# mstksg/hamilton

Measured on AMD Instinct MI355X. Metric: RK4 phase-space steps/sec (ensemble), higher is better.
Workload: dtype f64

## Files before the change

hamilton_amd/csrc/hamk_codegen.cpp:

```cpp
#include "hamk_internal.h"

#include <algorithm>
#include <array>
#include <cmath>
#include <cstdio>
#include <cstring>
#include <functional>
#include <map>
#include <set>
#include <sstream>

namespace hamk_host {

static std::string lit(double c) {
  if (std::isnan(c)) return "hamk::quiet_nan()";
  if (std::isinf(c)) return c > 0 ? "__builtin_inf()" : "(-__builtin_inf())";
  char buf[64];
  std::snprintf(buf, sizeof buf, "%a", c);
  std::string s(buf);
  if (c < 0 || std::signbit(c)) s = "(" + s + ")";
  return s;
}

static const char* unary_name(int op) {
// ... 414 lines not shown
        acc(p.a, 'a', aI + " * fa" + I + " + " + bI + " * (faa" + I + " * " + tanr(p.a) + " + fab" + I + " * " + tanr(p.b) + ")");
        acc(p.a, 'b', bI + " * fa" + I);
        acc(p.b, 'a', aI + " * fb" + I + " + " + bI + " * (fab" + I + " * " + tanr(p.a) + " + fbb" + I + " * " + tanr(p.b) + ")");
        acc(p.b, 'b', bI + " * fb" + I);
        break;
      case HAMK_OP_SIN: {
        const std::string sl = std::to_string(r.slot[i]);
        acc(p.a, 'a', aI + " * tcr.c[" + sl + "] - " + bI + " * tcr.s[" + sl + "] * " + tanr(p.a));
        acc(p.a, 'b', bI + " * tcr.c[" + sl + "]");
      } break;
      case HAMK_OP_COS: {
        const std::string sl = std::to_string(r.slot[i]);
        acc(p.a, 'a', "-(" + aI + " * tcr.s[" + sl + "] + " + bI + " * tcr.c[" + sl + "] * " + tanr(p.a) + ")");
        acc(p.a, 'b', "-(" + bI + " * tcr.s[" + sl + "])");
      } break;
      default:
        acc(p.a, 'a', aI + " * g" + I + " + " + bI + " * h" + I + " * " + tanr(p.a));
        acc(p.a, 'b', bI + " * g" + I);
        break;
    }
  }
  for (int j = 0; j < d.n; ++j) o << "    dT[" << j << "] = -aq" << j << "; (void)bq" << j << ";\n";
  o << "  }\n";
}

int distinct_jacobian_entries(const SystemDesc& d) {
  const int n = d.n, nops = (int)d.f_ops.size();
  enum : long long { ZERO = 0, ONE = 1 };
  std::map<std::array<long long, 4>, long long> table;
  long long next = 2;
  auto node = [&](long long kind, long long a, long long b, long long c) -> long long {
    const std::array<long long, 4> key = {kind, a, b, c};
    auto it = table.find(key);
    if (it != table.end()) return it->second;
    table[key] = next;
    return next++;
  };
  auto add = [&](long long a, long long b) { if (a == ZERO) return b; if (b == ZERO) return a; return node(1, std::min(a, b), std::max(a, b), 0); };
  auto neg = [&](long long a) { return a == ZERO ? (long long)ZERO : node(2, a, 0, 0); };
  auto scale = [&](long long factor_kind, long long factor_id, long long a) {
    if (a == ZERO) return (long long)ZERO;
    return node(3, factor_kind * (1LL << 40) + factor_id, a, 0);
  };
  std::vector<std::vector<long long>> g(nops, std::vector<long long>(n, ZERO));
  for (int i = 0; i < nops; ++i) {
    const hamk_op& p = d.f_ops[i];
    switch (p.op) {
      case HAMK_OP_CONST: break;
      case HAMK_OP_INPUT: g[i][p.a] = ONE; break;
      case HAMK_OP_ADD: for (int j = 0; j < n; ++j) g[i][j] = add(g[p.a][j], g[p.b][j]); break;
      case HAMK_OP_SUB: for (int j = 0; j < n; ++j) g[i][j] = add(g[p.a][j], neg(g[p.b][j])); break;
      case HAMK_OP_NEG: for (int j = 0; j < n; ++j) g[i][j] = neg(g[p.a][j]); break;
      case HAMK_OP_MUL: {
        const bool ca = d.f_ops[p.a].op == HAMK_OP_CONST, cb = d.f_ops[p.b].op == HAMK_OP_CONST;
        for (int j = 0; j < n; ++j) {
          const long long t1 = cb ? (long long)ZERO : scale(ca ? 5 : 4, ca ? (long long)std::hash<double>{}(d.f_ops[p.a].c) & ((1LL << 40) - 1) : p.a, g[p.b][j]);
          const long long t2 = ca ? (long long)ZERO : scale(cb ? 5 : 4, cb ? (long long)std::hash<double>{}(d.f_ops[p.b].c) & ((1LL << 40) - 1) : p.b, g[p.a][j]);
          g[i][j] = add(t1, t2);
        }
      } break;
      case HAMK_OP_DIV: case HAMK_OP_POW: case HAMK_OP_ATAN2:
        for (int j = 0; j < n; ++j) g[i][j] = (g[p.a][j] == ZERO && g[p.b][j] == ZERO) ? (long long)ZERO : node(6, i, g[p.a][j], g[p.b][j]);
        break;
      default:
        for (int j = 0; j < n; ++j) g[i][j] = scale(7 + p.op, p.a, g[p.a][j]);
        break;
    }
  }
  std::set<long long> distinct;
  for (int k = 0; k < d.m; ++k)
    for (int j = 0; j < n; ++j)
      if (g[d.f_outs[k]][j] != ZERO) distinct.insert(g[d.f_outs[k]][j]);
  return (int)distinct.size();
}

long long forward_gradient_work(const SystemDesc& d) {
  const int n = d.n, nops = (int)d.f_ops.size();
  std::vector<std::vector<char>> sup(nops, std::vector<char>(n, 0));
  auto count = [&](const std::vector<char>& v) { long long c = 0; for (char x : v) c += x; return c; };
  long long work = 0;
  for (int i = 0; i < nops; ++i) {
    const hamk_op& p = d.f_ops[i];
    if (p.op == HAMK_OP_CONST) continue;
    if (p.op == HAMK_OP_INPUT) { sup[i][p.a] = 1; continue; }
    if (is_binary(p.op)) {
      long long both = 0, any = 0;
      for (int j = 0; j < n; ++j) { const char a = sup[p.a][j], b = sup[p.b][j]; sup[i][j] = a | b; both += a & b; any += a | b; }
      const bool ca = d.f_ops[p.a].op == HAMK_OP_CONST, cb = d.f_ops[p.b].op == HAMK_OP_CONST;
      if (p.op == HAMK_OP_ADD || p.op == HAMK_OP_SUB) work += both;
      else if (ca || cb) work += any;
      else work += count(sup[p.a]) + count(sup[p.b]);
    } else {
      sup[i] = sup[p.a];
      work += (p.op == HAMK_OP_NEG) ? 0 : count(sup[i]) + 2;
    }
  }
  return work;
}

namespace {
typedef std::vector<std::pair<int, int>> Mono;
typedef std::map<Mono, double> Poly;
struct SymFail {};

Mono mono_mul(const Mono& a, const Mono& b) {
  Mono r; size_t i = 0, j = 0;
  while (i < a.size() || j < b.size()) {
    if (j >= b.size() || (i < a.size() && a[i].first < b[j].first)) r.push_back(a[i++]);
    else if (i >= a.size() || b[j].first < a[i].first) r.push_back(b[j++]);
    else { r.push_back({a[i].first, a[i].second + b[j].second}); ++i; ++j; }
  }
  return r;
}
void poly_add(Poly& a, const Poly& b, double f = 1.0) {
  for (const auto& t : b) { a[t.first] += f * t.second; }
  if (a.size() > 20000) throw SymFail{};
}
Poly poly_mul(const Poly& a, const Poly& b) {
  Poly r;
  if (a.size() * b.size() > 200000) throw SymFail{};
  for (const auto& x : a) for (const auto& y : b) r[mono_mul(x.first, y.first)] += x.second * y.second;
  return r;
}
Poly poly_const(double c) { Poly p; if (c != 0.0) p[Mono{}] = c; return p; }
Poly poly_var(int v) { Poly p; p[Mono{{v, 1}}] = 1.0; return p; }
Poly poly_reduce(const Poly& a, int n, int hi = 1 << 30) {
  Poly cur = a;
  for (bool again = true; again;) {
    again = false;
    Poly next;
    for (const auto& t : cur) {
      int at = -1;
      for (size_t i = 0; i < t.first.size(); ++i)
        if (t.first[i].first >= n && t.first[i].first < hi && ((t.first[i].first - n) & 1) == 0 && t.first[i].second >= 2) { at = (int)i; break; }
      if (at < 0) { next[t.first] += t.second; continue; }
      again = true;
      Mono rest = t.first;
      const int sv = rest[at].first;
      rest[at].second -= 2;
      if (rest[at].second == 0) rest.erase(rest.begin() + at);
      next[rest] += t.second;
      next[mono_mul(rest, Mono{{sv + 1, 2}})] -= t.second;
    }
    cur.swap(next);
    if (cur.size() > 20000) throw SymFail{};
  }
  return cur;
}
void poly_prune(Poly& p, double scale) {
  for (auto it = p.begin(); it != p.end();) it = (std::fabs(it->second) <= 8.0 * 2.220446049250313e-16 * scale) ? p.erase(it) : std::next(it);
}
double poly_abs_sum(const Poly& p) { double s = 0.0; for (const auto& t : p) s += std::fabs(t.second); return s; }

struct SymK {
  bool ok = false;
  int n = 0;
  std::vector<Poly> k;
  std::vector<Poly> dT;
  int vbase = 0;
  bool dt_ok = false;
  long long sym_ops = 0, num_ops = 0, dt_ops = 0;
};

SymK symbolic_mass_matrix(const SystemDesc& d, const std::vector<int>& slot_operand) {
  SymK out;
  const int n = d.n, m = d.m, nops = (int)d.f_ops.size();
  out.n = n;
  if (n > 7 || d.mapping != HAMK_MAP_LANE) return out;
  std::vector<int> slot_of(nops, -1);
  for (size_t k = 0; k < slot_operand.size(); ++k) if (slot_operand[k] >= 0) slot_of[(size_t)slot_operand[k]] = (int)k;
  try {
    std::vector<Poly> V(nops);
    std::vector<std::vector<Poly>> G(nops, std::vector<Poly>(n));
    for (int i = 0; i < nops; ++i) {
      const hamk_op& p = d.f_ops[i];
      switch (p.op) {
        case HAMK_OP_CONST: V[i] = poly_const(p.c); break;
        case HAMK_OP_INPUT: V[i] = poly_var(p.a); G[i][p.a] = poly_const(1.0); break;
        case HAMK_OP_ADD: V[i] = V[p.a]; poly_add(V[i], V[p.b]); for (int j = 0; j < n; ++j) { G[i][j] = G[p.a][j]; poly_add(G[i][j], G[p.b][j]); } break;
        case HAMK_OP_SUB: V[i] = V[p.a]; poly_add(V[i], V[p.b], -1.0); for (int j = 0; j < n; ++j) { G[i][j] = G[p.a][j]; poly_add(G[i][j], G[p.b][j], -1.0); } break;
        case HAMK_OP_NEG: poly_add(V[i], V[p.a], -1.0); for (int j = 0; j < n; ++j) poly_add(G[i][j], G[p.a][j], -1.0); break;
        case HAMK_OP_MUL:
          V[i] = poly_reduce(poly_mul(V[p.a], V[p.b]), n);
          for (int j = 0; j < n; ++j) {
            if (!G[p.b][j].empty()) poly_add(G[i][j], poly_mul(V[p.a], G[p.b][j]));
            if (!G[p.a][j].empty()) poly_add(G[i][j], poly_mul(G[p.a][j], V[p.b]));
            G[i][j] = poly_reduce(G[i][j], n);
          }
          break;
        case HAMK_OP_DIV: {
          if (d.f_ops[p.b].op != HAMK_OP_CONST || d.f_ops[p.b].c == 0.0) throw SymFail{};
          const double r = 1.0 / d.f_ops[p.b].c;
          poly_add(V[i], V[p.a], r); for (int j = 0; j < n; ++j) poly_add(G[i][j], G[p.a][j], r);
        } break;
        case HAMK_OP_POWI: {
          if (p.b < 0 || p.b > 6) throw SymFail{};
          Poly acc = poly_const(1.0), dacc;
          for (int e = 0; e < p.b; ++e) { dacc = acc; acc = poly_reduce(poly_mul(acc, V[p.a]), n); }
          V[i] = acc;
          if (p.b >= 1) for (int j = 0; j < n; ++j) if (!G[p.a][j].empty()) { Poly t = poly_mul(dacc, G[p.a][j]); poly_add(G[i][j], t, (double)p.b); G[i][j] = poly_reduce(G[i][j], n); }
        } break;
        case HAMK_OP_SIN: case HAMK_OP_COS: {
          const int k = slot_of[p.a];
          if (k < 0) throw SymFail{};
          const int sv = n + 2 * k, cv = sv + 1;
          const bool is_sin = p.op == HAMK_OP_SIN;
          V[i] = poly_var(is_sin ? sv : cv);
          for (int j = 0; j < n; ++j)
            if (!G[p.a][j].empty()) { Poly t = poly_mul(poly_var(is_sin ? cv : sv), G[p.a][j]); poly_add(G[i][j], t, is_sin ? 1.0 : -1.0); G[i][j] = poly_reduce(G[i][j], n); }
        } break;
        default: throw SymFail{};
      }
    }
    out.k.resize((size_t)n * (n + 1) / 2);
    size_t e = 0;
    for (int a = 0; a < n; ++a)
      for (int b = a; b < n; ++b, ++e) {
        Poly acc;
        double scale = 0.0;
        int both = 0;
        for (int k = 0; k < m; ++k) {
          const Poly& ga = G[d.f_outs[k]][a];
          const Poly& gb = G[d.f_outs[k]][b];
          if (ga.empty() || gb.empty()) continue;
          ++both;
          Poly t = poly_mul(ga, gb);
          scale += std::fabs(d.inertia[k]) * poly_abs_sum(t);
          poly_add(acc, t, d.inertia[k]);
        }
        acc = poly_reduce(acc, n);
        poly_prune(acc, scale);
        out.num_ops += 2LL * both;
        for (const auto& t : acc) {
          int deg = 0; for (const auto& vp : t.first) deg += vp.second;
          out.sym_ops += deg + ((std::fabs(t.second) != 1.0 && deg > 0) ? 1 : 0);
        }
        if (acc.size() > 1) out.sym_ops += (long long)acc.size() - 1;
        if (acc.size() > 24) throw SymFail{};
        out.k[e] = acc;
      }
    out.ok = out.sym_ops < out.num_ops;
    if (out.ok) {
      const int nslots = (int)slot_operand.size();
      out.vbase = n + 2 * nslots;
      auto dvar = [&](int var, int i) -> Poly {
        if (var < n) return (var == i) ? poly_const(1.0) : Poly();
        const int k = (var - n) / 2;
        const Poly& arg = G[slot_operand[(size_t)k]][i];
        if (arg.empty()) return Poly();
        Poly r = poly_mul(poly_var(((var - n) & 1) ? var - 1 : var + 1), arg);
        if ((var - n) & 1) { Poly neg; poly_add(neg, r, -1.0); return neg; }
        return r;
      };
      out.dT.assign((size_t)n, Poly());
      bool fits = true;
      for (int i = 0; i < n && fits; ++i) {
        Poly acc;
        double scale = 0.0;
        size_t e2 = 0;
        for (int a = 0; a < n; ++a)
          for (int b = a; b < n; ++b, ++e2) {
            const double w = (a == b) ? -0.5 : -1.0;
            for (const auto& t : out.k[e2]) {
              for (size_t f = 0; f < t.first.size(); ++f) {
                const Poly dv = dvar(t.first[f].first, i);
                if (dv.empty()) continue;
                Mono rest = t.first;
                const double pw = (double)rest[f].second;
                rest[f].second -= 1;
                if (rest[f].second == 0) rest.erase(rest.begin() + (long)f);
                Mono vv = (a == b) ? Mono{{out.vbase + a, 2}} : Mono{{out.vbase + a, 1}, {out.vbase + b, 1}};
                Poly term; term[mono_mul(rest, vv)] = w * pw * t.second;
                Poly prod = poly_mul(term, dv);
                scale += poly_abs_sum(prod);
                poly_add(acc, prod);
              }
            }
          }
        acc = poly_reduce(acc, n, out.vbase);
        poly_prune(acc, scale);
        for (const auto& t : acc) { int deg = 0; for (const auto& vp : t.first) deg += vp.second; out.dt_ops += deg + 1; }
        if (acc.size() > 64) fits = false;
        out.dT[(size_t)i] = acc;
      }
      out.dt_ok = fits && out.dt_ops <= 12LL * n;
    }
  } catch (const SymFail&) { out.ok = false; out.dt_ok = false; }
  return out;
}

static std::string sym_poly_expr(const Poly& p, int n, int vbase) {
  std::ostringstream x;
  bool first = true;
  for (const auto& t : p) {
    std::ostringstream f;
    bool unit = true;
    for (const auto& vp : t.first)
      for (int r = 0; r < vp.second; ++r) {
        f << (unit ? "" : " * ");
        unit = false;
        if (vp.first < n) f << "q[" << vp.first << "]";
        else if (vp.first >= vbase) f << "v[" << (vp.first - vbase) << "]";
        else f << "tc." << (((vp.first - n) & 1) ? "c" : "s") << "[" << (vp.first - n) / 2 << "]";
      }
    if (!first) x << " + ";
    first = false;
    if (unit) x << lit(t.second);
    else if (t.second == 1.0) x << f.str();
    else x << lit(t.second) << " * " << f.str();
  }
  if (first) x << "0.0";
  return x.str();
}

void emit_symbolic_dt(std::ostringstream& o, const SymK& sk) {
  o << "  // dT/dq = -1/2 v^T (dK/dq) v from the symbolic K (" << sk.dt_ops << " operations): no second-order sweep of f\n";
  o << "  template <class TC> __device__ __forceinline__ static void dT_sym(const double (&q)[N], const double (&v)[N], const TC& tc, double (&dT)[N]) {\n";
  for (int i = 0; i < sk.n; ++i) o << "    dT[" << i << "] = " << sym_poly_expr(sk.dT[(size_t)i], sk.n, sk.vbase) << ";\n";
  o << "  }\n";
}

void emit_symbolic_k(std::ostringstream& o, const SymK& sk) {
  const int n = sk.n;
  o << "  // K = J^T M J derived symbolically (sin^2 + cos^2 = 1 applied; " << sk.sym_ops << " operations against " << sk.num_ops << " for the numerical sum)\n";
  o << "  template <class TC> __device__ __forceinline__ static void mass_matrix_sym(const double (&q)[N], const TC& tc, double (&K)[N][N]) {\n";
  size_t e = 0;
  for (int a = 0; a < n; ++a)
    for (int b = a; b < n; ++b, ++e) {
      std::ostringstream x;
      bool first = true;
      for (const auto& t : sk.k[e]) {
        std::ostringstream f;
        bool unit = true;
        for (const auto& vp : t.first)
          for (int r = 0; r < vp.second; ++r) {
            f << (unit ? "" : " * ");
            unit = false;
            if (vp.first < n) f << "q[" << vp.first << "]";
            else f << "tc." << (((vp.first - n) & 1) ? "c" : "s") << "[" << (vp.first - n) / 2 << "]";
          }
        if (!first) x << " + ";
        first = false;
        if (unit) x << lit(t.second);
        else if (t.second == 1.0) x << f.str();
        else x << lit(t.second) << " * " << f.str();
      }
      if (first) x << "0.0";
      o << "    K[" << a << "][" << b << "] = " << x.str() << ";\n";
      if (a != b) o << "    K[" << b << "][" << a << "] = K[" << a << "][" << b << "];\n";
    }
  o << "  }\n";
}
}

bool symbolic_rhs_applies(const SystemDesc& d0) {
  SystemDesc d = d0;
  d.mapping = HAMK_MAP_LANE;
  if (!d.k_symbolic) return false;
  std::vector<int> slot_of(d.f_ops.size(), -1), slot_operand;
  for (const hamk_op& p : d.f_ops)
    if ((p.op == HAMK_OP_SIN || p.op == HAMK_OP_COS) && slot_of[(size_t)p.a] < 0) { slot_of[(size_t)p.a] = (int)slot_operand.size(); slot_operand.push_back(p.a); }
  const SymK sk = symbolic_mass_matrix(d, slot_operand);
  return sk.ok && sk.dt_ok;
}

std::string generate_source(const SystemDesc& d) {
  std::ostringstream o;
  o << "// generated by libhamk (hamk_codegen.cpp) from the expression tape of one System " << d.m << " " << d.n << "\n";
  if (d.rk4_min_waves > 1 || d.wave) o << "#define HAMK_RK4_MIN_WAVES " << d.rk4_min_waves << "\n#define HAMK_RK4_MIN_WAVES_BIG " << d.rk4_min_waves << "\n";
  if (d.wave && d.n > 32 && d.rk4_min_waves > 1) o << "#define HAMK_RKF_MIN_WAVES " << d.rk4_min_waves << "\n";
  o << "#define HAMK_USE_LUT " << d.use_lut << "\n";
  o << "#define HAMK_K_REASSOC " << (d.k_reassoc ? 1 : 0) << "\n";
  if (d.rk4_park && !d.wave) o << "#define HAMK_RK4_PARK 1\n";
  if (d.mapping == HAMK_MAP_QUAD) o << "#define HAMK_QUAD_RKF_PARK " << (d.rkf_park ? 1 : 0) << "\n";
  if (d.mapping == HAMK_MAP_LANE && d.trig_const_vgpr && d.use_lut != 0) o << "#define HAMK_TRIG_CONST_VGPR 1\n";
  if (d.mapping == HAMK_MAP_LANE && d.pair_rows) o << "#define HAMK_PAIR_ROWS 1\n";
  if (d.mapping == HAMK_MAP_LANE && d.rkf_two_waves)
    o << "#define HAMK_RKF_MIN_WAVES_LANE 2\n#define HAMK_RKF_LDS_BUDGET 36\n#define HAMK_RKF_ROWS_IN_REGS 1\n";
  o << "#ifdef HAMK_HOST_EMULATION\nstatic const double hamk_trig_lut_init[1024] = {\n#else\n__device__ const double hamk_trig_lut_init[1024] = {\n#endif\n";
  for (int i = 0; i < 512; ++i) {
    const long double a = (long double)i * (2.0L * 3.14159265358979323846264338327950288L / 512.0L);
    o << "  " << lit((double)sinl(a)) << ", " << lit((double)cosl(a)) << (i == 511 ? "\n" : ",\n");
  }
  o << "};\n";
  const bool quad = d.mapping == HAMK_MAP_QUAD;
  o << (d.wave ? "#include \"hamk_wave.hpp\"\n\n" : (quad ? "#include \"hamk_quad.hpp\"\n\n" : "#include \"hamk_device.hpp\"\n\n"));
  o << "struct HamkSys {\n";
  o << "  static constexpr int N = " << d.n << ";\n";
  o << "  static constexpr int M = " << d.m << ";\n";
  o << "  static constexpr bool U_CART = " << (d.u_space == HAMK_U_CARTESIAN ? "true" : "false") << ";\n";
  o << "  static constexpr bool MODE_H = " << (d.mode_h ? "true" : "false") << ";\n";
  o << "  static constexpr bool RK4_STAGE_LOOP = " << (d.rk4_stage_loop ? "true" : "false") << ";\n";
  o << "  static constexpr bool RKF_STAGE_LOOP = " << (d.rkf_stage_loop ? "true" : "false") << ";\n";
  o << "  static constexpr bool MODE_R = " << (d.mode_r ? "true" : "false") << ";\n";
  bool inertia_pos = true;
  for (double w : d.inertia) inertia_pos = inertia_pos && (w > 0.0);
  o << "  static constexpr bool INERTIA_POS = " << (inertia_pos ? "true" : "false") << ";\n";
  o << "  static constexpr bool QUAD_DENSE = " << ((quad && d.quad_dense) ? "true" : "false") << ";\n";
  o << "  __device__ __forceinline__ static constexpr double inertia(int k) {\n";
  o << "    constexpr double w[M] = {";
  for (int k = 0; k < d.m; ++k) o << (k ? ", " : "") << lit(d.inertia[k]);
  o << "};\n    return w[k];\n  }\n";
  o << "  template <class A, int TRIG, class TC> __device__ __forceinline__ static void coords(const A (&in)[N], A (&x)[M], TC& tc) {\n";
  std::vector<int> slot_operand;
  auto mark_f = [&] { mark_outputs(d.f_ops.size(), d.f_outs.data(), d.m); g_emit_unshare_scales = d.mapping == HAMK_MAP_QUAD && d.quad_dense; };
  auto mark_u = [&] { mark_outputs(d.u_ops.size(), &d.u_out, 1); g_emit_unshare_scales = false; };
  mark_f();
  const int ntrig_f = emit_body(o, d.f_ops.data(), (int)d.f_ops.size(), "f", nullptr, nullptr, "tc", &slot_operand);
  for (int k = 0; k < d.m; ++k) o << "    x[" << k << "] = hamk::lift<A>(" << value_name(d.f_ops, "f", d.f_outs[k]) << ");\n";
  o << "  }\n";
  const int nu = d.u_space == HAMK_U_CARTESIAN ? d.m : d.n;
  o << "  template <class A, int TRIG, class TC> __device__ __forceinline__ static A potential(const A (&in)[" << nu << "], TC& tc) {\n";
  mark_u();
  const int ntrig_u = emit_body(o, d.u_ops.data(), (int)d.u_ops.size(), "u");
  o << "    return hamk::lift<A>(" << value_name(d.u_ops, "u", d.u_out) << ");\n";
  o << "  }\n";
  {
    std::vector<int> f_slot_of_input(d.n, -1);
    bool any = false;
    if (d.u_space == HAMK_U_GENERALIZED) {
      for (int k = 0; k < ntrig_f; ++k) {
        const int opi = slot_operand[k];
        if (opi >= 0 && d.f_ops[opi].op == HAMK_OP_INPUT) f_slot_of_input[d.f_ops[opi].a] = k;
      }
      for (const hamk_op& p : d.u_ops)
        if ((p.op == HAMK_OP_SIN || p.op == HAMK_OP_COS) && d.u_ops[p.a].op == HAMK_OP_INPUT && f_slot_of_input[d.u_ops[p.a].a] >= 0) any = true;
    }
    o << "  static constexpr bool U_SHARES_F_TRIG = " << (any ? "true" : "false") << ";\n";
    o << "  template <class A, int TRIG, class TC, class TCF> __device__ __forceinline__ static A potential_after_f(const A (&in)[" << nu
      << "], TC& tc, TCF& tcf) {\n";
    if (any) {
      mark_u();
      emit_body(o, d.u_ops.data(), (int)d.u_ops.size(), "u", nullptr, nullptr, "tc", nullptr, "TRIG", &f_slot_of_input);
      o << "    return hamk::lift<A>(" << value_name(d.u_ops, "u", d.u_out) << ");\n";
    } else {
      o << "    return potential<A, TRIG>(in, tc);\n";
    }
    o << "  }\n";
  }
  o << "  template <class A, int TRIG, class IN, class TC, class Sink> __device__ __forceinline__ static void coords_sink(const IN& in, TC& tc, Sink& sink) {\n";
  std::vector<std::vector<int>> sink_outs(d.f_ops.size());
  for (int k = 0; k < d.m; ++k) sink_outs[d.f_outs[k]].push_back(k);
  std::vector<int> put_order;
  mark_f();
  emit_body(o, d.f_ops.data(), (int)d.f_ops.size(), "f", &sink_outs, nullptr, "tc", nullptr, "TRIG", nullptr, &put_order);
  o << "  }\n";
  o << "  template <class A, int TRIG, class IN, class TC, class TCU, class Sink> __device__ __forceinline__ static A coords_sink_u(const IN& in, TC& tc, TCU& tcu, Sink& sink) {\n";
  mark_f();
  emit_body(o, d.f_ops.data(), (int)d.f_ops.size(), "f", &sink_outs);
  {
    std::vector<std::string> u_in;
    if (d.u_space == HAMK_U_CARTESIAN) for (int k = 0; k < d.m; ++k) u_in.push_back(value_name(d.f_ops, "f", d.f_outs[k]));
    else for (int j = 0; j < d.n; ++j) u_in.push_back("in[" + std::to_string(j) + "]");
    mark_u();
    emit_body(o, d.u_ops.data(), (int)d.u_ops.size(), "u", nullptr, &u_in, "tcu", nullptr, "hamk::TRIG_FULL");
    o << "    return hamk::lift<A>(" << value_name(d.u_ops, "u", d.u_out, &u_in) << ");\n";
  }
  o << "  }\n";
  o << "  __device__ __forceinline__ static constexpr int trig_input(int slot) {\n    constexpr int w[" << (ntrig_f > 0 ? ntrig_f : 1) << "] = {";
  bool all_inputs = ntrig_f > 0;
  for (int k = 0; k < ntrig_f; ++k) {
    const int opi = slot_operand[k];
    const int inp = (opi >= 0 && d.f_ops[opi].op == HAMK_OP_INPUT) ? d.f_ops[opi].a : -1;
    if (inp < 0) all_inputs = false;
    o << (k ? ", " : "") << inp;
  }
  if (ntrig_f == 0) o << "-1";
  o << "};\n    return w[slot];\n  }\n";
  o << "  static constexpr bool TRIG_ALL_INPUTS = " << (all_inputs ? "true" : "false") << ";\n";
  if (d.wave) {
    const int nf = (int)d.f_ops.size();
    std::vector<int> lo(nf, 1 << 30), hi(nf, -1);
    for (int i = 0; i < nf; ++i) {
      const hamk_op& p = d.f_ops[i];
      if (p.op == HAMK_OP_CONST) continue;
      if (p.op == HAMK_OP_INPUT) { lo[i] = hi[i] = p.a; continue; }
      lo[i] = lo[p.a]; hi[i] = hi[p.a];
      if (is_binary(p.op)) { lo[i] = std::min(lo[i], lo[p.b]); hi[i] = std::max(hi[i], hi[p.b]); }
    }
    auto table = [&](const char* name, const std::vector<int>& w) {
      o << "  __device__ __forceinline__ static constexpr int " << name << "(int k) {\n    constexpr int w[" << w.size() << "] = {";
      for (size_t k = 0; k < w.size(); ++k) o << (k ? ", " : "") << w[k];
      o << "};\n    return w[k];\n  }\n";
    };
    std::vector<int> dlo(d.m), dhi(d.m);
    for (int k = 0; k < d.m; ++k) { const int v = d.f_outs[k]; dlo[k] = hi[v] < 0 ? -1 : lo[v]; dhi[k] = hi[v]; }
    table("dep_lo", dlo);
    table("dep_hi", dhi);
    table("seq_out", put_order);
  }
  emit_reverse(o, d);
  {
    const SymK sk = d.k_symbolic ? symbolic_mass_matrix(d, slot_operand) : SymK();
    o << "  static constexpr bool HAS_SYM_K = " << (sk.ok ? "true" : "false") << ";\n";
    if (sk.ok) emit_symbolic_k(o, sk);
    else o << "  template <class TC> __device__ __forceinline__ static void mass_matrix_sym(const double (&)[N], const TC&, double (&)[N][N]) {}\n";
    o << "  static constexpr bool HAS_SYM_DT = " << ((sk.ok && sk.dt_ok) ? "true" : "false") << ";\n";
    if (sk.ok && sk.dt_ok) emit_symbolic_dt(o, sk);
    else o << "  template <class TC> __device__ __forceinline__ static void dT_sym(const double (&)[N], const double (&)[N], const TC&, double (&)[N]) {}\n";
  }
  o << "  static constexpr int NTRIG_F = " << ntrig_f << ";\n";
  o << "  static constexpr int NTRIG_U = " << ntrig_u << ";\n";
  o << "};\n\n";
  o << (d.wave ? "HAMK_INSTANTIATE_WAVE(HamkSys)\n" : (quad ? "HAMK_INSTANTIATE_QUAD(HamkSys)\n" : "HAMK_INSTANTIATE(HamkSys)\n"));
  return o.str();
}

}
```

hamilton_amd/csrc/hamk_device.hpp:

```cpp
#pragma once
#ifndef __HIPCC_RTC__
#include <hip/hip_runtime.h>
#endif

#define HAMK_DEV __device__ __forceinline__
#ifndef HAMK_JET_REASSOC
#define HAMK_JET_REASSOC 1
#endif
#ifndef HAMK_K_REASSOC
#define HAMK_K_REASSOC 1
#endif
#ifndef HAMK_RKF_LDS_BUDGET
#define HAMK_RKF_LDS_BUDGET 76
#endif
#ifndef HAMK_RKF_ROWS_IN_REGS
#define HAMK_RKF_ROWS_IN_REGS 0
#endif
#ifndef HAMK_PAIR_ROWS
#define HAMK_PAIR_ROWS 0
#endif
#if HAMK_PAIR_ROWS
#define HAMK_ROW_AT(j) ((((j) >> 1) * 512) + ((j) & 1))
#define HAMK_ROW_LANE (2 * threadIdx.x)
#else
// ... 724 lines not shown
#pragma unroll
  for (int j = 0; j < S::N; ++j) {
    qa[j].v = q[j];
#pragma unroll
    for (int i = 0; i < S::N; ++i) qa[j].d[i] = (i == j) ? 1.0 : 0.0;
  }
}

template <class S, class A> HAMK_DEV void mass_matrix(const A (&x)[S::M], double (&K)[S::N][S::N]) {
#if HAMK_K_REASSOC
#pragma clang fp reassociate(on)
#pragma unroll
  for (int a = 0; a < S::N; ++a)
#pragma unroll
    for (int b = a; b < S::N; ++b) {
      double acc = 0.0;
#pragma unroll
      for (int k = 0; k < S::M; ++k) acc += (S::inertia(k) * x[k].d[a]) * x[k].d[b];
      K[a][b] = acc;
      K[b][a] = acc;
    }
#else
#pragma unroll
  for (int a = 0; a < S::N; ++a)
#pragma unroll
    for (int b = a; b < S::N; ++b) {
      double acc = 0.0;
#pragma unroll
      for (int k = 0; k < S::M; ++k) acc = fma(S::inertia(k) * x[k].d[a], x[k].d[b], acc);
      K[a][b] = acc;
      K[b][a] = acc;
    }
#endif
}

template <class S> HAMK_DEV void grad_potential(const Jet1<S::N> (&qj)[S::N], const Jet1<S::N> (&xj)[S::M],
                                                double (&gU)[S::N], double& U, TrigCache<S::NTRIG_F>& tcf) {
  Jet1<S::N> u;
  TrigCache<S::NTRIG_U> tu;
  if constexpr (S::U_CART) u = S::template potential<Jet1<S::N>, TRIG_FULL>(xj, tu);
  else u = S::template potential_after_f<Jet1<S::N>, TRIG_FULL>(qj, tu, tcf);
  U = u.v;
#pragma unroll
  for (int i = 0; i < S::N; ++i) gU[i] = u.d[i];
}

template <class S> HAMK_DEV void momenta(const double (&q)[S::N], const double (&qd)[S::N], double (&p)[S::N]) {
  constexpr int N = S::N, M = S::M;
  Jet1<N> qj[N], xj[M];
  TrigCache<S::NTRIG_F> tc;
  seed1<S>(q, qj);
  S::template coords<Jet1<N>, TRIG_FULL>(qj, xj, tc);
  double w[M];
#pragma unroll
  for (int k = 0; k < M; ++k) {
    double a = 0.0;
#pragma unroll
    for (int i = 0; i < N; ++i) a = fma(xj[k].d[i], qd[i], a);
    w[k] = S::inertia(k) * a;
  }
#pragma unroll
  for (int i = 0; i < N; ++i) {
    double a = 0.0;
#pragma unroll
    for (int k = 0; k < M; ++k) a = fma(xj[k].d[i], w[k], a);
    p[i] = a;
  }
}

template <class S> HAMK_DEV void velocities(const double (&q)[S::N], const double (&p)[S::N], double (&qd)[S::N], int& st) {
  constexpr int N = S::N, M = S::M;
  Jet1<N> qj[N], xj[M];
  TrigCache<S::NTRIG_F> tc;
  seed1<S>(q, qj);
  S::template coords<Jet1<N>, TRIG_FULL>(qj, xj, tc);
  double K[N][N];
  if constexpr (S::HAS_SYM_K) S::mass_matrix_sym(q, tc, K); else mass_matrix<S>(xj, K);
  solve_spd<N, S::INERTIA_POS>(K, p, qd, st);
}

template <class S> HAMK_DEV double potential_value(const double (&q)[S::N]) {
  TrigCache<S::NTRIG_U> tu;
  if constexpr (S::U_CART) {
    double x[S::M];
    TrigCache<S::NTRIG_F> tc;
    S::template coords<double, TRIG_FULL>(q, x, tc);
    return S::template potential<double, TRIG_FULL>(x, tu);
  } else {
    return S::template potential<double, TRIG_FULL>(q, tu);
  }
}

#ifndef HAMK_TRIG_BURST
#define HAMK_TRIG_BURST 1
#endif
template <class S, class TC> HAMK_DEV void trig_burst_lut(const double (&q)[S::N], TC& tc) {
  constexpr int NS = (S::NTRIG_F > 0) ? S::NTRIG_F : 1;
  const auto kc = lut_consts(tc, 0);
  double r[NS], sa[NS], ca[NS];
  int idx[NS];
#pragma unroll
  for (int k = 0; k < NS; ++k) {
    const double x = q[S::trig_input(k)];
    const double kk = rint(x * kc.inv_step);
    double rr = fma(-kk, kc.w0, x);
    rr = fma(-kk, kc.w1, rr);
    r[k] = fma(-kk, kc.w2, rr);
    idx[k] = ((int)kk) & (HAMK_LUT_N - 1);
  }
#pragma unroll
  for (int k = 0; k < NS; ++k) { sa[k] = HAMK_LUT[2 * idx[k]]; ca[k] = HAMK_LUT[2 * idx[k] + 1]; }
#ifndef HAMK_HOST_EMULATION
  __builtin_amdgcn_sched_barrier(0);
#endif
  double sd[NS], cm1[NS];
#pragma unroll
  for (int k = 0; k < NS; ++k) {
    const double z = r[k] * r[k];
    const double ps = fma(kc.s5, z, kc.s3);
    sd[k] = fma(r[k] * z, ps, r[k]);
    double pc = fma(kc.c6, z, kc.c4);
    pc = fma(pc, z, -0.5);
    cm1[k] = z * pc;
  }
#ifndef HAMK_HOST_EMULATION
  __builtin_amdgcn_sched_barrier(0);
#endif
#pragma unroll
  for (int k = 0; k < NS; ++k) {
#if HAMK_ROTATE_HORNER
    tc.s[k] = fma(ca[k], sd[k], fma(sa[k], cm1[k], sa[k]));
    tc.c[k] = fma(-sa[k], sd[k], fma(ca[k], cm1[k], ca[k]));
#else
    tc.s[k] = sa[k] + fma(sa[k], cm1[k], ca[k] * sd[k]);
    tc.c[k] = ca[k] + fma(ca[k], cm1[k], -(sa[k] * sd[k]));
#endif
  }
#ifndef HAMK_PROBE_NO_SLOWPATH
#pragma unroll
  for (int k = 0; k < NS; ++k) {
    const double x = q[S::trig_input(k)];
    if (!(fabs(x) < kc.lim)) { tc.s[k] = ::sin(x); tc.c[k] = ::cos(x); }
  }
#endif
}

template <class S, bool MODE_H, int TRIG_IN = TRIG_FULL, bool BURST_OK = true>
HAMK_DEV void ham_eqs(const double (&q)[S::N], const double (&p)[S::N], double (&dq)[S::N], double (&dp)[S::N], int& st,
                      TrigCache<S::NTRIG_F>& tc) {
  constexpr int N = S::N, M = S::M;
  constexpr bool BURST = (HAMK_TRIG_BURST == 2 || (HAMK_TRIG_BURST == 1 && BURST_OK)) && TRIG_IN == TRIG_LUT && S::TRIG_ALL_INPUTS && S::NTRIG_F >= 2;
  if constexpr (BURST) trig_burst_lut<S>(q, tc);
  constexpr int TRIG = BURST ? TRIG_REUSE : TRIG_IN;
  double K[N][N], gU[N], U, v[N], dT[N];
  if constexpr (S::HAS_SYM_K && S::HAS_SYM_DT) {
    Jet1<N> qj[N], xj[M];
    seed1<S>(q, qj);
    S::template coords<Jet1<N>, TRIG>(qj, xj, tc);
    S::mass_matrix_sym(q, tc, K);
    solve_spd<N, S::INERTIA_POS>(K, p, v, st);
    grad_potential<S>(qj, xj, gU, U, tc);
    S::dT_sym(q, v, tc, dT);
  } else if constexpr (MODE_H) {
    JetH<N> qh[N], xh[M];
#pragma unroll
    for (int j = 0; j < N; ++j) {
      qh[j] = lift<JetH<N>>(q[j]);
      qh[j].d[j] = 1.0;
    }
    S::template coords<JetH<N>, TRIG>(qh, xh, tc);
    Jet1<N> qj[N], xj[M];
    seed1<S>(q, qj);
#pragma unroll
    for (int k = 0; k < M; ++k) {
      xj[k].v = xh[k].v;
#pragma unroll
      for (int i = 0; i < N; ++i) xj[k].d[i] = xh[k].d[i];
    }
    if constexpr (S::HAS_SYM_K) S::mass_matrix_sym(q, tc, K); else mass_matrix<S>(xj, K);
    solve_spd<N, S::INERTIA_POS>(K, p, v, st);
    grad_potential<S>(qj, xj, gU, U, tc);
#pragma unroll
    for (int i = 0; i < N; ++i) dT[i] = 0.0;
#pragma unroll
    for (int k = 0; k < M; ++k) {
      double jv = 0.0;
#pragma unroll
      for (int j = 0; j < N; ++j) jv = fma(xh[k].d[j], v[j], jv);
      const double uk = S::inertia(k) * jv;
#pragma unroll
      for (int i = 0; i < N; ++i) {
        double hv = 0.0;
#pragma unroll
        for (int j = 0; j < N; ++j) hv = fma(xh[k].h[(i <= j) ? hidx<N>(i, j) : hidx<N>(j, i)], v[j], hv);
        dT[i] = fma(-uk, hv, dT[i]);
      }
    }
  } else {
    Jet1<N> qj[N], xj[M];
    seed1<S>(q, qj);
    S::template coords<Jet1<N>, TRIG>(qj, xj, tc);
    if constexpr (S::HAS_SYM_K) S::mass_matrix_sym(q, tc, K); else mass_matrix<S>(xj, K);
    solve_spd<N, S::INERTIA_POS>(K, p, v, st);
    grad_potential<S>(qj, xj, gU, U, tc);
    if constexpr (S::MODE_R) {
      S::dT_reverse(q, v, tc, dT);
    } else {
      Jet2<N> q2[N], x2[M];
#pragma unroll
      for (int j = 0; j < N; ++j) {
        q2[j] = lift<Jet2<N>>(q[j]);
        q2[j].d[j] = 1.0;
        q2[j].dv = v[j];
      }
      S::template coords<Jet2<N>, TRIG_REUSE>(q2, x2, tc);
#pragma unroll
      for (int i = 0; i < N; ++i) dT[i] = 0.0;
#pragma unroll
      for (int k = 0; k < M; ++k) {
        const double uk = S::inertia(k) * x2[k].dv;
#pragma unroll
        for (int i = 0; i < N; ++i) dT[i] = fma(-uk, x2[k].dd[i], dT[i]);
      }
    }
  }
#pragma unroll
  for (int i = 0; i < N; ++i) {
    dq[i] = v[i];
    dp[i] = -(dT[i] + gU[i]);
  }
}

#ifndef HAMK_TRIG_FEW_MAX
#define HAMK_TRIG_FEW_MAX 4
#endif
template <class S> struct StageTrig {
  static constexpr bool few = (S::NTRIG_F >= 1 && S::NTRIG_F <= HAMK_TRIG_FEW_MAX);
  static constexpr bool lut = (HAMK_USE_LUT != 0) && (S::NTRIG_F >= 1);
#ifdef HAMK_NO_INCR
  static constexpr bool on = false;
#else
  static constexpr bool on = few && (HAMK_USE_LUT != 1);
#endif
  static constexpr int anchor = lut ? TRIG_LUT : (few ? TRIG_ANCHOR : TRIG_FULL);
  static constexpr int incr = lut ? TRIG_LUT : (few ? TRIG_INCR : TRIG_FULL);
  static constexpr int dyn = on ? TRIG_DYN : (lut ? TRIG_LUT : TRIG_FULL);
  static constexpr bool burst_rk4 = (S::N <= 7) || (S::N >= 14);
};

template <class S, int TRIG = TRIG_FULL, bool BURST_OK = true>
HAMK_DEV void rhs(const double (&y)[2 * S::N], double (&dy)[2 * S::N], int& st, TrigCache<S::NTRIG_F>& tc) {
  constexpr int N = S::N;
  double q[N], p[N], dq[N], dp[N];
#pragma unroll
  for (int i = 0; i < N; ++i) { q[i] = y[i]; p[i] = y[N + i]; }
  ham_eqs<S, S::MODE_H, TRIG, BURST_OK>(q, p, dq, dp, st, tc);
#pragma unroll
  for (int i = 0; i < N; ++i) { dy[i] = dq[i]; dy[N + i] = dp[i]; }
}

HAMK_DEV bool is_nonfinite_bits(double x) {
  unsigned int hi = (unsigned int)__double2hiint(x);
#ifdef HAMK_HOST_EMULATION
  asm volatile("" : "+r"(hi));
#else
  asm volatile("" : "+v"(hi));
#endif
  return (hi & 0x7ff00000u) == 0x7ff00000u;
}


template <class S> HAMK_DEV double energy(const double (&y)[2 * S::N], int& st) {
  constexpr int N = S::N;
  double q[N], p[N], v[N];
#pragma unroll
  for (int j = 0; j < N; ++j) { q[j] = y[j]; p[j] = y[N + j]; }
  velocities<S>(q, p, v, st);
  double t = 0.0;
#pragma unroll
  for (int j = 0; j < N; ++j) t = fma(v[j], p[j], t);
  return fma(0.5, t, potential_value<S>(q));
}

template <class S>
HAMK_DEV void rk4_body(double* __restrict__ q, double* __restrict__ p, i64 B, double dt, int nsteps, double drift_tol,
                       int* __restrict__ status) {
  constexpr int N = S::N, D = 2 * N;
  if constexpr (StageTrig<S>::lut) lut_load();
  const i64 i = (i64)blockIdx.x * blockDim.x + threadIdx.x;
  if (i >= B) return;
  double y[D];
#pragma unroll
  for (int j = 0; j < N; ++j) { y[j] = q[(i64)j * B + i]; y[N + j] = p[(i64)j * B + i]; }
  int st = 0;
  TrigCache<S::NTRIG_F> tc;
  const double h2 = 0.5 * dt, h6 = dt * (1.0 / 6.0), h3 = dt * (1.0 / 3.0);
  double H0 = 0.0;
  if (drift_tol > 0.0) H0 = energy<S>(y, st);
  if constexpr (S::RK4_STAGE_LOOP && HAMK_RK4_PARK) {
    __shared__ __attribute__((aligned(16))) double park[2 * D * 256];
    double* py = park + HAMK_ROW_LANE;
    double* pa = park + D * 256 + HAMK_ROW_LANE;
#pragma unroll
    for (int j = 0; j < D; ++j) { py[HAMK_ROW_AT(j)] = y[j]; pa[HAMK_ROW_AT(j)] = y[j]; }
    double k[D];
#pragma unroll
    for (int j = 0; j < D; ++j) k[j] = 0.0;
#pragma unroll 1
    for (int it = 0; it < 4 * nsteps; ++it) {
      const int sg = it & 3;
      const double a = (sg == 0) ? 0.0 : ((sg == 3) ? dt : h2);
      const double b = (sg == 0 || sg == 3) ? h6 : h3;
      double yt[D];
#pragma unroll
      for (int j = 0; j < D; ++j) yt[j] = fma(a, k[j], py[HAMK_ROW_AT(j)]);
      tc.mode = sg;
      if (sg >= 2) tc.mode = 5 - sg;
#ifndef HAMK_HOST_EMULATION
      __builtin_amdgcn_sched_barrier(0);
#endif
      rhs<S, StageTrig<S>::dyn, StageTrig<S>::burst_rk4>(yt, k, st, tc);
#ifndef HAMK_HOST_EMULATION
      __builtin_amdgcn_sched_barrier(0);
#endif
      if (sg == 3) {
#pragma unroll
        for (int j = 0; j < D; ++j) { const double v = fma(b, k[j], pa[HAMK_ROW_AT(j)]); pa[HAMK_ROW_AT(j)] = v; py[HAMK_ROW_AT(j)] = v; }
      } else {
#pragma unroll
        for (int j = 0; j < D; ++j) pa[HAMK_ROW_AT(j)] = fma(b, k[j], pa[HAMK_ROW_AT(j)]);
      }
    }
#pragma unroll
    for (int j = 0; j < D; ++j) y[j] = py[HAMK_ROW_AT(j)];
  } else if constexpr (S::RK4_STAGE_LOOP) {
    double k[D], acc[D];
#pragma unroll
    for (int j = 0; j < D; ++j) { k[j] = 0.0; acc[j] = y[j]; }
#pragma unroll 1
    for (int it = 0; it < 4 * nsteps; ++it) {
      const int sg = it & 3;
      const double a = (sg == 0) ? 0.0 : ((sg == 3) ? dt : h2);
      const double b = (sg == 0 || sg == 3) ? h6 : h3;
      double yt[D];
#pragma unroll
      for (int j = 0; j < D; ++j) yt[j] = fma(a, k[j], y[j]);
      tc.mode = sg;
      if (sg >= 2) tc.mode = 5 - sg;
      rhs<S, StageTrig<S>::dyn, StageTrig<S>::burst_rk4>(yt, k, st, tc);
#pragma unroll
      for (int j = 0; j < D; ++j) acc[j] = fma(b, k[j], acc[j]);
      if (sg == 3) {
#pragma unroll
        for (int j = 0; j < D; ++j) y[j] = acc[j];
      }
    }
// ... 799 lines not shown
```

Baseline: 108.2 billion.

## Derive potential gradient symbolically and skip jet sweep of coordinates and potential

Extends the host-side symbolic engine to push the potential U through the polynomial form of the coordinate map and emit a closed-form gU_sym kernel helper. When K, dT and gU are all available symbolically, ham_eqs evaluates coordinates in plain doubles, used only to fill the trig cache, instead of first-order jets, and computes grad U directly. This removes the dual-number sweep over f and U per RHS evaluation. In exchange the generated polynomials may be longer and the numerics change through pruning. It also refactors the polynomial sweep and expression printer into shared helpers.

```diff
diff --git a/hamilton_amd/csrc/hamk_codegen.cpp b/hamilton_amd/csrc/hamk_codegen.cpp
--- a/hamilton_amd/csrc/hamk_codegen.cpp
+++ b/hamilton_amd/csrc/hamk_codegen.cpp
@@ -590,6 +590,92 @@
 }
 double poly_abs_sum(const Poly& p) { double s = 0.0; for (const auto& t : p) s += std::fabs(t.second); return s; }
 
+template <class Slot>
+void poly_sweep(const std::vector<hamk_op>& ops, int n, const std::vector<Poly>& inV, const std::vector<std::vector<Poly>>& inG, Slot slot,
+                std::vector<Poly>& V, std::vector<std::vector<Poly>>& G, std::vector<std::vector<double>>& GS) {
+  const int nops = (int)ops.size();
+  V.assign((size_t)nops, Poly());
+  G.assign((size_t)nops, std::vector<Poly>((size_t)n));
+  GS.assign((size_t)nops, std::vector<double>((size_t)n, 0.0));
+  std::vector<double> VS((size_t)nops, 0.0);
+  for (int i = 0; i < nops; ++i) {
+    const hamk_op& p = ops[(size_t)i];
+    switch (p.op) {
+      case HAMK_OP_CONST: V[i] = poly_const(p.c); VS[i] = std::fabs(p.c); break;
+      case HAMK_OP_INPUT:
+        V[i] = inV[(size_t)p.a]; G[i] = inG[(size_t)p.a]; VS[i] = poly_abs_sum(V[i]);
+        for (int j = 0; j < n; ++j) GS[i][j] = poly_abs_sum(G[i][j]);
+        break;
+      case HAMK_OP_ADD: V[i] = V[p.a]; poly_add(V[i], V[p.b]); for (int j = 0; j < n; ++j) { G[i][j] = G[p.a][j]; poly_add(G[i][j], G[p.b][j]); GS[i][j] = GS[p.a][j] + GS[p.b][j]; } VS[i] = VS[p.a] + VS[p.b]; break;
+      case HAMK_OP_SUB: V[i] = V[p.a]; poly_add(V[i], V[p.b], -1.0); for (int j = 0; j < n; ++j) { G[i][j] = G[p.a][j]; poly_add(G[i][j], G[p.b][j], -1.0); GS[i][j] = GS[p.a][j] + GS[p.b][j]; } VS[i] = VS[p.a] + VS[p.b]; break;
+      case HAMK_OP_NEG: poly_add(V[i], V[p.a], -1.0); for (int j = 0; j < n; ++j) { poly_add(G[i][j], G[p.a][j], -1.0); GS[i][j] = GS[p.a][j]; } VS[i] = VS[p.a]; break;
+      case HAMK_OP_MUL:
+        V[i] = poly_reduce(poly_mul(V[p.a], V[p.b]), n);
+        VS[i] = VS[p.a] * VS[p.b];
+        for (int j = 0; j < n; ++j) {
+          if (!G[p.b][j].empty()) poly_add(G[i][j], poly_mul(V[p.a], G[p.b][j]));
+          if (!G[p.a][j].empty()) poly_add(G[i][j], poly_mul(G[p.a][j], V[p.b]));
+          G[i][j] = poly_reduce(G[i][j], n);
+          GS[i][j] = VS[p.a] * GS[p.b][j] + GS[p.a][j] * VS[p.b];
+        }
+        break;
+      case HAMK_OP_DIV: {
+        if (ops[(size_t)p.b].op != HAMK_OP_CONST || ops[(size_t)p.b].c == 0.0) throw SymFail{};
+        const double r = 1.0 / ops[(size_t)p.b].c;
+        poly_add(V[i], V[p.a], r); for (int j = 0; j < n; ++j) { poly_add(G[i][j], G[p.a][j], r); GS[i][j] = std::fabs(r) * GS[p.a][j]; }
+        VS[i] = std::fabs(r) * VS[p.a];
+      } break;
+      case HAMK_OP_POWI: {
+        if (p.b < 0 || p.b > 6) throw SymFail{};
+        Poly acc = poly_const(1.0), dacc;
+        for (int e = 0; e < p.b; ++e) { dacc = acc; acc = poly_reduce(poly_mul(acc, V[p.a]), n); }
+        V[i] = acc;
+        VS[i] = std::pow(VS[p.a], (double)p.b);
+        if (p.b >= 1) for (int j = 0; j < n; ++j) if (!G[p.a][j].empty()) {
+          Poly t = poly_mul(dacc, G[p.a][j]); poly_add(G[i][j], t, (double)p.b); G[i][j] = poly_reduce(G[i][j], n);
+          GS[i][j] = (double)p.b * std::pow(VS[p.a], (double)(p.b - 1)) * GS[p.a][j];
+        }
+      } break;
+      case HAMK_OP_SIN: case HAMK_OP_COS: {
+        const int k = slot(p.a, V[p.a]);
+        if (k < 0) throw SymFail{};
+        const int sv = n + 2 * k, cv = sv + 1;
+        const bool is_sin = p.op == HAMK_OP_SIN;
+        V[i] = poly_var(is_sin ? sv : cv);
+        VS[i] = 1.0;
+        for (int j = 0; j < n; ++j)
+          if (!G[p.a][j].empty()) { Poly t = poly_mul(poly_var(is_sin ? cv : sv), G[p.a][j]); poly_add(G[i][j], t, is_sin ? 1.0 : -1.0); G[i][j] = poly_reduce(G[i][j], n); GS[i][j] = GS[p.a][j]; }
+      } break;
+      default: throw SymFail{};
+    }
+  }
+}
+
+struct PolyNames { int n = 0, vbase = 1 << 30; };
+static std::string poly_expr(const Poly& p, const PolyNames& nm) {
+  std::ostringstream x;
+  bool first = true;
+  for (const auto& t : p) {
+    std::ostringstream f;
+    bool unit = true;
+    for (const auto& vp : t.first)
+      for (int r = 0; r < vp.second; ++r) {
+        f << (unit ? "" : " * ");
+        unit = false;
+        if (vp.first < nm.n) f << "q[" << vp.first << "]";
+        else if (vp.first >= nm.vbase) f << "v[" << (vp.first - nm.vbase) << "]";
+        else f << "tc." << (((vp.first - nm.n) & 1) ? "c" : "s") << "[" << (vp.first - nm.n) / 2 << "]";
+      }
+    if (!first) x << " + ";
+    first = false;
+    if (unit) x << lit(t.second);
+    else if (t.second == 1.0) x << f.str();
+    else x << lit(t.second) << " * " << f.str();
+  }
+  if (first) x << "0.0";
+  return x.str();
+}
+
 struct SymK {
   bool ok = false;
   int n = 0;
@@ -597,6 +683,8 @@
   std::vector<Poly> dT;
   int vbase = 0;
   bool dt_ok = false;
+  std::vector<Poly> gU;
+  bool gu_ok = false;
   long long sym_ops = 0, num_ops = 0, dt_ops = 0;
 };
 
@@ -605,50 +693,17 @@
   const int n = d.n, m = d.m, nops = (int)d.f_ops.size();
   out.n = n;
   if (n > 7 || d.mapping != HAMK_MAP_LANE) return out;
-  std::vector<int> slot_of(nops, -1);
-  for (size_t k = 0; k < slot_operand.size(); ++k) if (slot_operand[k] >= 0) slot_of[(size_t)slot_operand[k]] = (int)k;
   try {
-    std::vector<Poly> V(nops);
-    std::vector<std::vector<Poly>> G(nops, std::vector<Poly>(n));
-    for (int i = 0; i < nops; ++i) {
-      const hamk_op& p = d.f_ops[i];
-      switch (p.op) {
-        case HAMK_OP_CONST: V[i] = poly_const(p.c); break;
-        case HAMK_OP_INPUT: V[i] = poly_var(p.a); G[i][p.a] = poly_const(1.0); break;
-        case HAMK_OP_ADD: V[i] = V[p.a]; poly_add(V[i], V[p.b]); for (int j = 0; j < n; ++j) { G[i][j] = G[p.a][j]; poly_add(G[i][j], G[p.b][j]); } break;
-        case HAMK_OP_SUB: V[i] = V[p.a]; poly_add(V[i], V[p.b], -1.0); for (int j = 0; j < n; ++j) { G[i][j] = G[p.a][j]; poly_add(G[i][j], G[p.b][j], -1.0); } break;
-        case HAMK_OP_NEG: poly_add(V[i], V[p.a], -1.0); for (int j = 0; j < n; ++j) poly_add(G[i][j], G[p.a][j], -1.0); break;
-        case HAMK_OP_MUL:
-          V[i] = poly_reduce(poly_mul(V[p.a], V[p.b]), n);
-          for (int j = 0; j < n; ++j) {
-            if (!G[p.b][j].empty()) poly_add(G[i][j], poly_mul(V[p.a], G[p.b][j]));
-            if (!G[p.a][j].empty()) poly_add(G[i][j], poly_mul(G[p.a][j], V[p.b]));
-            G[i][j] = poly_reduce(G[i][j], n);
-          }
-          break;
-        case HAMK_OP_DIV: {
-          if (d.f_ops[p.b].op != HAMK_OP_CONST || d.f_ops[p.b].c == 0.0) throw SymFail{};
-          const double r = 1.0 / d.f_ops[p.b].c;
-          poly_add(V[i], V[p.a], r); for (int j = 0; j < n; ++j) poly_add(G[i][j], G[p.a][j], r);
-        } break;
-        case HAMK_OP_POWI: {
-          if (p.b < 0 || p.b > 6) throw SymFail{};
-          Poly acc = poly_const(1.0), dacc;
-          for (int e = 0; e < p.b; ++e) { dacc = acc; acc = poly_reduce(poly_mul(acc, V[p.a]), n); }
-          V[i] = acc;
-          if (p.b >= 1) for (int j = 0; j < n; ++j) if (!G[p.a][j].empty()) { Poly t = poly_mul(dacc, G[p.a][j]); poly_add(G[i][j], t, (double)p.b); G[i][j] = poly_reduce(G[i][j], n); }
-        } break;
-        case HAMK_OP_SIN: case HAMK_OP_COS: {
-          const int k = slot_of[p.a];
-          if (k < 0) throw SymFail{};
-          const int sv = n + 2 * k, cv = sv + 1;
-          const bool is_sin = p.op == HAMK_OP_SIN;
-          V[i] = poly_var(is_sin ? sv : cv);
-          for (int j = 0; j < n; ++j)
-            if (!G[p.a][j].empty()) { Poly t = poly_mul(poly_var(is_sin ? cv : sv), G[p.a][j]); poly_add(G[i][j], t, is_sin ? 1.0 : -1.0); G[i][j] = poly_reduce(G[i][j], n); }
-        } break;
-        default: throw SymFail{};
-      }
+    std::vector<Poly> V;
+    std::vector<std::vector<Poly>> G;
+    std::vector<std::vector<double>> GS;
+    {
+      std::vector<Poly> inV((size_t)n);
+      std::vector<std::vector<Poly>> inG((size_t)n, std::vector<Poly>((size_t)n));
+      for (int j = 0; j < n; ++j) { inV[(size_t)j] = poly_var(j); inG[(size_t)j][(size_t)j] = poly_const(1.0); }
+      std::vector<int> slot_of(nops, -1);
+      for (size_t k = 0; k < slot_operand.size(); ++k) if (slot_operand[k] >= 0) slot_of[(size_t)slot_operand[k]] = (int)k;
+      poly_sweep(d.f_ops, n, inV, inG, [&](int operand, const Poly&) { return slot_of[(size_t)operand]; }, V, G, GS);
     }
     out.k.resize((size_t)n * (n + 1) / 2);
     size_t e = 0;
@@ -722,69 +777,64 @@
         out.dT[(size_t)i] = acc;
       }
       out.dt_ok = fits && out.dt_ops <= 12LL * n;
+      if (out.dt_ok) {
+        try {
+          const bool cart = d.u_space == HAMK_U_CARTESIAN;
+          const int nin = cart ? m : n;
+          std::vector<Poly> inV((size_t)nin);
+          std::vector<std::vector<Poly>> inG((size_t)nin, std::vector<Poly>((size_t)n));
+          for (int k = 0; k < nin; ++k) {
+            if (cart) { inV[(size_t)k] = V[(size_t)d.f_outs[k]]; inG[(size_t)k] = G[(size_t)d.f_outs[k]]; }
+            else { inV[(size_t)k] = poly_var(k); inG[(size_t)k][(size_t)k] = poly_const(1.0); }
+          }
+          std::vector<Poly> UV;
+          std::vector<std::vector<Poly>> UG;
+          std::vector<std::vector<double>> US;
+          poly_sweep(d.u_ops, n, inV, inG, [&](int, const Poly& arg) {
+            for (int k = 0; k < nslots; ++k) if (slot_operand[(size_t)k] >= 0 && V[(size_t)slot_operand[(size_t)k]] == arg) return k;
+            return -1;
+          }, UV, UG, US);
+          out.gU.assign((size_t)n, Poly());
+          bool short_enough = true;
+          for (int i = 0; i < n; ++i) {
+            Poly g = poly_reduce(UG[(size_t)d.u_out][(size_t)i], n);
+            poly_prune(g, US[(size_t)d.u_out][(size_t)i]);
+            if (g.size() > 64) short_enough = false;
+            out.gU[(size_t)i] = g;
+          }
+          out.gu_ok = short_enough;
+        } catch (const SymFail&) { out.gu_ok = false; }
+      }
     }
   } catch (const SymFail&) { out.ok = false; out.dt_ok = false; }
   return out;
 }
 
-static std::string sym_poly_expr(const Poly& p, int n, int vbase) {
-  std::ostringstream x;
-  bool first = true;
-  for (const auto& t : p) {
-    std::ostringstream f;
-    bool unit = true;
-    for (const auto& vp : t.first)
-      for (int r = 0; r < vp.second; ++r) {
-        f << (unit ? "" : " * ");
-        unit = false;
-        if (vp.first < n) f << "q[" << vp.first << "]";
-        else if (vp.first >= vbase) f << "v[" << (vp.first - vbase) << "]";
-        else f << "tc." << (((vp.first - n) & 1) ? "c" : "s") << "[" << (vp.first - n) / 2 << "]";
-      }
-    if (!first) x << " + ";
-    first = false;
-    if (unit) x << lit(t.second);
-    else if (t.second == 1.0) x << f.str();
-    else x << lit(t.second) << " * " << f.str();
-  }
-  if (first) x << "0.0";
-  return x.str();
-}
-
 void emit_symbolic_dt(std::ostringstream& o, const SymK& sk) {
+  PolyNames nm; nm.n = sk.n; nm.vbase = sk.vbase;
   o << "  // dT/dq = -1/2 v^T (dK/dq) v from the symbolic K (" << sk.dt_ops << " operations): no second-order sweep of f\n";
   o << "  template <class TC> __device__ __forceinline__ static void dT_sym(const double (&q)[N], const double (&v)[N], const TC& tc, double (&dT)[N]) {\n";
-  for (int i = 0; i < sk.n; ++i) o << "    dT[" << i << "] = " << sym_poly_expr(sk.dT[(size_t)i], sk.n, sk.vbase) << ";\n";
+  for (int i = 0; i < sk.n; ++i) o << "    dT[" << i << "] = " << poly_expr(sk.dT[(size_t)i], nm) << ";\n";
+  o << "  }\n";
+}
+
+void emit_symbolic_gu(std::ostringstream& o, const SymK& sk) {
+  PolyNames nm; nm.n = sk.n;
+  o << "  // grad U of the polynomial U . f: no first-order sweep of f and U\n";
+  o << "  template <class TC> __device__ __forceinline__ static void gU_sym(const double (&q)[N], const TC& tc, double (&gU)[N]) {\n";
+  for (int i = 0; i < sk.n; ++i) o << "    gU[" << i << "] = " << poly_expr(sk.gU[(size_t)i], nm) << ";\n";
   o << "  }\n";
 }
 
 void emit_symbolic_k(std::ostringstream& o, const SymK& sk) {
   const int n = sk.n;
+  PolyNames nm; nm.n = n;
   o << "  // K = J^T M J derived symbolically (sin^2 + cos^2 = 1 applied; " << sk.sym_ops << " operations against " << sk.num_ops << " for the numerical sum)\n";
   o << "  template <class TC> __device__ __forceinline__ static void mass_matrix_sym(const double (&q)[N], const TC& tc, double (&K)[N][N]) {\n";
   size_t e = 0;
   for (int a = 0; a < n; ++a)
     for (int b = a; b < n; ++b, ++e) {
-      std::ostringstream x;
-      bool first = true;
-      for (const auto& t : sk.k[e]) {
-        std::ostringstream f;
-        bool unit = true;
-        for (const auto& vp : t.first)
-          for (int r = 0; r < vp.second; ++r) {
-            f << (unit ? "" : " * ");
-            unit = false;
-            if (vp.first < n) f << "q[" << vp.first << "]";
-            else f << "tc." << (((vp.first - n) & 1) ? "c" : "s") << "[" << (vp.first - n) / 2 << "]";
-          }
-        if (!first) x << " + ";
-        first = false;
-        if (unit) x << lit(t.second);
-        else if (t.second == 1.0) x << f.str();
-        else x << lit(t.second) << " * " << f.str();
-      }
-      if (first) x << "0.0";
-      o << "    K[" << a << "][" << b << "] = " << x.str() << ";\n";
+      o << "    K[" << a << "][" << b << "] = " << poly_expr(sk.k[e], nm) << ";\n";
       if (a != b) o << "    K[" << b << "][" << a << "] = K[" << a << "][" << b << "];\n";
     }
   o << "  }\n";
@@ -936,6 +986,10 @@
     o << "  static constexpr bool HAS_SYM_DT = " << ((sk.ok && sk.dt_ok) ? "true" : "false") << ";\n";
     if (sk.ok && sk.dt_ok) emit_symbolic_dt(o, sk);
     else o << "  template <class TC> __device__ __forceinline__ static void dT_sym(const double (&)[N], const double (&)[N], const TC&, double (&)[N]) {}\n";
+    const bool gu = sk.ok && sk.dt_ok && sk.gu_ok;
+    o << "  static constexpr bool HAS_SYM_GU = " << (gu ? "true" : "false") << ";\n";
+    if (gu) emit_symbolic_gu(o, sk);
+    else o << "  template <class TC> __device__ __forceinline__ static void gU_sym(const double (&)[N], const TC&, double (&)[N]) {}\n";
   }
   o << "  static constexpr int NTRIG_F = " << ntrig_f << ";\n";
   o << "  static constexpr int NTRIG_U = " << ntrig_u << ";\n";
diff --git a/hamilton_amd/csrc/hamk_device.hpp b/hamilton_amd/csrc/hamk_device.hpp
--- a/hamilton_amd/csrc/hamk_device.hpp
+++ b/hamilton_amd/csrc/hamk_device.hpp
@@ -900,13 +900,21 @@
   constexpr bool BURST = (HAMK_TRIG_BURST == 2 || (HAMK_TRIG_BURST == 1 && BURST_OK)) && TRIG_IN == TRIG_LUT && S::TRIG_ALL_INPUTS && S::NTRIG_F >= 2;
   if constexpr (BURST) trig_burst_lut<S>(q, tc);
   constexpr int TRIG = BURST ? TRIG_REUSE : TRIG_IN;
-  double K[N][N], gU[N], U, v[N], dT[N];
-  if constexpr (S::HAS_SYM_K && S::HAS_SYM_DT) {
+  double K[N][N], gU[N], v[N], dT[N];
+  if constexpr (S::HAS_SYM_K && S::HAS_SYM_DT && S::HAS_SYM_GU) {
+    double x[M];
+    S::template coords<double, TRIG>(q, x, tc);
+    S::mass_matrix_sym(q, tc, K);
+    solve_spd<N, S::INERTIA_POS>(K, p, v, st);
+    S::gU_sym(q, tc, gU);
+    S::dT_sym(q, v, tc, dT);
+  } else if constexpr (S::HAS_SYM_K && S::HAS_SYM_DT) {
     Jet1<N> qj[N], xj[M];
     seed1<S>(q, qj);
     S::template coords<Jet1<N>, TRIG>(qj, xj, tc);
     S::mass_matrix_sym(q, tc, K);
     solve_spd<N, S::INERTIA_POS>(K, p, v, st);
+    double U;
     grad_potential<S>(qj, xj, gU, U, tc);
     S::dT_sym(q, v, tc, dT);
   } else if constexpr (MODE_H) {
@@ -927,6 +935,7 @@
     }
     if constexpr (S::HAS_SYM_K) S::mass_matrix_sym(q, tc, K); else mass_matrix<S>(xj, K);
     solve_spd<N, S::INERTIA_POS>(K, p, v, st);
+    double U;
     grad_potential<S>(qj, xj, gU, U, tc);
 #pragma unroll
     for (int i = 0; i < N; ++i) dT[i] = 0.0;
@@ -950,6 +959,7 @@
     S::template coords<Jet1<N>, TRIG>(qj, xj, tc);
     if constexpr (S::HAS_SYM_K) S::mass_matrix_sym(q, tc, K); else mass_matrix<S>(xj, K);
     solve_spd<N, S::INERTIA_POS>(K, p, v, st);
+    double U;
     grad_potential<S>(qj, xj, gU, U, tc);
     if constexpr (S::MODE_R) {
       S::dT_reverse(q, v, tc, dT);
```

Measured after the change: 111.0 billion, median of 6. 2.5% higher.
